# kamimrcht/ELECTOR

Measured on NVIDIA B200. Metric: triplets_per_sec, higher is better.
Workload: dtype s16x2 (packed halfword integer SIMD; int32 for scores beyond 16 bits)

## Files before the change

elector_b200/csrc/poa_dual.cuh:

```cuda
#pragma once
#include "poa_kernel.cuh"
#include "poa_packed.cuh"

namespace elector {

EL_HD uint32_t pk_select(uint32_t fresh, uint32_t old, uint32_t take) { return (fresh & take) | (old & ~take); }
EL_HD uint32_t pk_prmt(uint32_t a, uint32_t b, uint32_t sel) {
#ifdef __CUDA_ARCH__
  uint32_t r;
  asm("prmt.b32 %0, %1, %2, %3;" : "=r"(r) : "r"(a), "r"(b), "r"(sel));
  return r;
#else
  const uint64_t ab = ((uint64_t)b << 32) | a;
  uint32_t r = 0;
  for (int i = 0; i < 4; ++i) {
    const uint32_t n = (sel >> (4 * i)) & 0xfu;
    uint32_t byte = (uint32_t)(ab >> (8 * (n & 7u))) & 0xffu;
    if (n & 8u) byte = (byte & 0x80u) ? 0xffu : 0u;
    r |= byte << (8 * i);
  }
  return r;
#endif
}

enum : uint32_t { NM_REF = 1u << 7, NM_COR = 1u << 15, NM_MERGE = 1u << 23, NM_FINAL = 1u, NM_REFWINS = 2u };

struct Phase2D : Phase2<false> {
  static constexpr int kSetWords = 1;
  static EL_HD void put_row0(uint32_t *p, int bS, int bG) { p[R2_BS * 32] = pk2(kBiasP + bS, kBiasP + bG); }
  static EL_HD void put_shape(uint32_t *p, uint32_t ra) {
    p[R2_BG * 32] = ((ra & NF_REF) ? NM_REF : 0u) | ((ra & NF_COR) ? NM_COR : 0u) | ((ra & (NF_VIRT | NF_TWO)) ? NM_MERGE : 0u) |
                    ((ra & NF_FINAL) ? NM_FINAL : 0u) | (((ra & NF_VIRT) && !(ra & NF_PREDC)) ? NM_REFWINS : 0u) | ((ra & 0xffu) << 24);
  }
  EL_HDN int prepare(const uint16_t *nodes, int nx) const { return prepare_nodes(*this, nodes, nx); }

  template <int R, bool REF_SECOND>
  static EL_HD void merge(uint32_t (&Sr)[R], uint32_t (&Gr)[R], const uint32_t (&Sc)[R], const uint32_t (&Gc)[R], uint32_t &hr, uint32_t hc,
                          uint32_t take, uint32_t &oM, uint32_t &oX) {
    const uint32_t hm = REF_SECOND ? pk_maxs_flag(hc, hr, oM, 1u, 0u) : pk_maxs_flag(hr, hc, oM, 1u, 0u);
    if (take & 0xffffu) hr = hm;
#pragma unroll
    for (int k = 0; k < R; ++k) {
      const uint32_t bMl = 4u << (2 * k), bMh = R + k + 1 < kBand ? 4u << (2 * (R + k)) : 0u;
      const uint32_t bXl = 1u << (2 * k), bXh = 1u << (2 * (R + k));
      const uint32_t ms = REF_SECOND ? pk_maxs_flag(Sc[k], Sr[k], oM, bMl, bMh) : pk_maxs_flag(Sr[k], Sc[k], oM, bMl, bMh);
      const uint32_t mx = REF_SECOND ? pk_maxs_flag(Gc[k], Gr[k], oX, bXl, bXh) : pk_maxs_flag(Gr[k], Gc[k], oX, bXl, bXh);
      Sr[k] = pk_select(ms, Sr[k], take);
      Gr[k] = pk_select(mx, Gr[k], take);
    }
  }

  template <int R>
  EL_HDN void band(int nx, int ly, int b, bool last, int &best, int &best_j) const {
    constexpr uint32_t kLowMoves = ~0u << (32 - 2 * R);
    constexpr uint32_t kLowOrdM = (4u << (2 * R)) - 1u;
    constexpr uint32_t kLowOrdX = (1u << (2 * R)) - 1u;
    const int r0 = b * kBand;
    PackedConsts pc;
    pc.set(sc);
    uint32_t y2[R], Sr[R], Gr[R], Sc[R], Gc[R];
#pragma unroll
    for (int k = 0; k < R; ++k) {
      y2[k] = ((uint32_t)fs.code_at(Lp->f_unc, r0 + k) | ((uint32_t)fs.code_at(Lp->f_unc, r0 + R + k) << 16)) * 0x0101u;
      Sr[k] = Sc[k] = pk2(kBiasP + sc.virt_S(r0 + k), kBiasP + sc.virt_S(r0 + R + k));
      Gr[k] = Gc[k] = pk2(kBiasP + sc.virt_G(r0 + k), kBiasP + sc.virt_G(r0 + R + k));
    }
    uint32_t hr = (uint32_t)(kBiasP + sc.virt_S(r0 - 1)), hc = hr;
    const int rr = ly - 1 - r0;
    const bool lowrow = rr < R;
    uint32_t *p = rec(0);
    const int32_t step = (int32_t)(Lp->rec_words * 32);
    const int32_t o_bs = (int32_t)(R2_BS * 32) - step, o_mv = (int32_t)((R2_MOVES + (uint32_t)b) * 32) - step;
    uint32_t mr = 0, mc = 0, mg = 0, x2 = 0, nm_h = 0;
    uint32_t d7 = 0, g7 = 0, mlo = 0, ordM_lo = 0, ordX_lo = 0;
    uint32_t nm = p[R2_BG * 32], bsg = p[R2_BS * 32];
    uint32_t nm_n = p[step + R2_BG * 32], bsg_n = p[step + R2_BS * 32];
    for (int j = 0; j <= nx; ++j, p += step) {
      const uint32_t nm_n2 = p[2 * step + R2_BG * 32], bsg_n2 = p[2 * step + R2_BS * 32];
      if (j >= nx) nm = 0;
      mr = pk_prmt(mr, nm, 0x10ccu);
      mc = pk_prmt(mc, nm, 0x10ddu);
      mg = pk_prmt(mg, nm, 0x10eeu);
      x2 = pk_prmt(x2, nm, 0x1077u);
      if (mg) {
        const bool low = mg & 0xffffu;
        const uint32_t ram = low ? 0u : (p - step)[R2_NODE * 32];
        uint32_t oM = 0, oX = 0;
        if ((low ? nm : nm_h) & NM_REFWINS) merge<R, true>(Sr, Gr, Sc, Gc, hr, hc, mg, oM, oX);
        else merge<R, false>(Sr, Gr, Sc, Gc, hr, hc, mg, oM, oX);
        if (mg & 0xffffu) { ordM_lo = oM & kLowOrdM; ordX_lo = oX & kLowOrdX; }
        else {
          uint32_t *po = scr.at(Lp->o_ord + ((ram >> NF_SLOT_SHIFT) * Lp->ord_bands + (uint32_t)b) * 2);
          po[0] = ordM_lo | (oM & ~kLowOrdM);
          po[32] = ordX_lo | (oX & ~kLowOrdX);
        }
      }
      const uint32_t diag0 = pk_prmt(pk_select(hr, hc, mr), d7, 0x5410u);
      const uint32_t up0 = pk_prmt(bsg, g7, 0x5432u);
      d7 = pk_select(Sr[R - 1], Sc[R - 1], mr);
      uint32_t mv = 0, diag = diag0, up = up0, s = 0, g = 0;
#pragma unroll
      for (int k = 0; k < R; ++k) {
        const uint32_t pS = pk_select(Sr[k], Sc[k], mr), pG = pk_select(Gr[k], Gc[k], mr);
        const uint32_t t = pk_minu(x2 ^ y2[k], pc.mis2);
        const uint32_t M = diag - t;
        const uint32_t gap = pk_maxs_flag(up, pG, mv, 1u << (2 * (kBand - 1 - k)), 1u << (2 * (kBand - 1 - R - k)));
        s = pk_maxs_flag(gap, M, mv, 2u << (2 * (kBand - 1 - k)), 2u << (2 * (kBand - 1 - R - k)));
        g = pk_addmaxs(M, pc.nopen2, gap - pc.ext2);
        Sr[k] = pk_select(s, Sr[k], mr); Sc[k] = pk_select(s, Sc[k], mc);
        Gr[k] = pk_select(g, Gr[k], mr); Gc[k] = pk_select(g, Gc[k], mc);
        diag = pS; up = g;
      }
      g7 = g;
      hr = pk_select(bsg, hr, mr);
      hc = pk_select(bsg, hc, mc);
      if (j > 0) {
        if (!last) p[o_bs] = pk_prmt(s, g, 0x7632u);
        st_stream(p + o_mv, (mlo & kLowMoves) | (mv & ~kLowMoves));
      }
      mlo = mv;
      if (last && ((lowrow ? nm : nm_h) & NM_FINAL)) {
        const int kk = lowrow ? rr : rr - R;
        uint32_t v = pk_select(Sr[0], Sc[0], mr);
#pragma unroll
        for (int k = 1; k < R; ++k) if (kk == k) v = pk_select(Sr[k], Sc[k], mr);
        const int sf = (int)(lowrow ? v & 0xffffu : v >> 16) - kBiasP;
        if (sf > best) { best = sf; best_j = lowrow ? j : j - 1; }
      }
      nm_h = nm;
      nm = nm_n; bsg = bsg_n;
      nm_n = nm_n2; bsg_n = bsg_n2;
    }
  }

  mutable const uint16_t *p1n = nullptr;
  EL_HDN int fuse_emit(const AlignBits &al, int n1, int lu, const RowSink &out) const {
    const uint8_t *sym = sc.tab->sym;
    int col = 0, ix = 0, iy = 0;
    uint32_t w0 = 0, w1 = 0, w2 = 0;
    uint32_t ra0 = n1 > 0 ? p1n[0] : 0u, ra1 = n1 > 1 ? p1n[1] : 0u, ra2 = n1 > 2 ? p1n[2] : 0u, ra3 = n1 > 3 ? p1n[3] : 0u;
    while (ix < n1 || iy < lu) {
      const bool two = ix + 1 < n1 && (ra1 & NF_SAMERING);
      const bool xa = ix < n1 && (al.x_at(ix) || (two && al.x_at(ix + 1)));
      const bool ya = iy < lu && ((fs.w(al.oy + (uint32_t)(iy >> 5)) >> (iy & 31)) & 1u);
      const bool yonly = iy < lu && !ya && (ix >= n1 || xa);
      const bool takey = yonly || xa;
      const uint32_t rb = two ? (ra0 | ra1) : ra0;
      const uint32_t rl = (ra0 & NF_REF) ? ra0 : ra1, cl = (ra0 & NF_COR) ? ra0 : ra1;
      const uint32_t rc = (rb & NF_REF) ? (uint32_t)sym[rl & 31u] : (uint32_t)'.';
      const uint32_t cc = (rb & NF_COR) ? (uint32_t)sym[cl & 31u] : (uint32_t)'.';
      const uint32_t yc = sym[(fs.w(Lp->f_unc + (uint32_t)(iy >> 2)) >> ((iy & 3) * 8)) & 31u];
      const int sh = (col & 3) * 8;
      w0 |= (yonly ? (uint32_t)'.' : rc) << sh;
      w1 |= (yonly ? (uint32_t)'.' : cc) << sh;
      w2 |= (takey ? yc : (uint32_t)'.') << sh;
      if ((col & 3) == 3) { st_stream(out.r0 + (col >> 2), w0); st_stream(out.r1 + (col >> 2), w1); st_stream(out.r2 + (col >> 2), w2); w0 = w1 = w2 = 0; }
      ++col;
      iy += takey;
      if (!yonly) {
        const int adv = two ? 2 : 1;
        ix += adv;
        if (two) { ra0 = ra2; ra1 = ra3; ra2 = ix + 2 < n1 ? p1n[ix + 2] : 0u; ra3 = ix + 3 < n1 ? p1n[ix + 3] : 0u; }
        else { ra0 = ra1; ra1 = ra2; ra2 = ra3; ra3 = ix + 3 < n1 ? p1n[ix + 3] : 0u; }
      }
    }
    if (col & 3) { st_stream(out.r0 + (col >> 2), w0); st_stream(out.r1 + (col >> 2), w1); st_stream(out.r2 + (col >> 2), w2); }
    return col;
  }

  EL_HDN int dp(int nx, int ly, int &best_j) const {
    const int nb = (ly + kBand - 1) / kBand;
    int best = -999999;
    best_j = -1;
    for (int b = 0; b < nb - 1; ++b) band<8>(nx, ly, b, false, best, best_j);
    if (ly - (nb - 1) * kBand <= 8) band<4>(nx, ly, nb - 1, true, best, best_j);
    else band<8>(nx, ly, nb - 1, true, best, best_j);
    return best;
  }

  EL_HDN int align_window(const uint16_t *p1, int n1, const uint8_t *unc, int lu, int &s2, AlignBits &al) const {
    p1n = p1;
    for (int k = 0; k < n1; k += 64) prefetch_l1(p1 + k);
    fs.pack_codes(sc.tab, unc, lu, Lp->f_unc);
    EL_TICK(*this, 1);
    const int nrings = prepare(p1, n1);
    EL_TICK(*this, 2);
    int bj;
    s2 = dp(n1, lu, bj);
    EL_TICK(*this, 3);
    traceback(n1, lu, bj, al);
    EL_TICK(*this, 4);
    return columns_of(nrings, lu, al.nmatch);
  }
};

}
```

elector_b200/csrc/poa_kernel.cuh:

```cuda
#pragma once
#include <cuda_runtime.h>
#include <stddef.h>
#include <stdint.h>

namespace elector {

constexpr int kBand = 16;

#define EL_WARP_FULL 0xffffffffu
#define EL_HD __host__ __device__ __forceinline__
#define EL_HDN __host__ __device__

EL_HD uint32_t cdiv_u(uint32_t a, uint32_t b) { return (a + b - 1) / b; }
EL_HD uint32_t max_u(uint32_t a, uint32_t b) { return a > b ? a : b; }

enum : uint32_t { R1_BS = 0, R1_BG = 1, R1_MOVES = 2 };
enum : uint32_t { R2_NODE = 0, R2_BS = 1, R2_BG = 2, R2_PRED = 3, R2_MOVES = 4 };

struct Layout1 {
  uint32_t o_nodes;
  uint32_t rec_words;
  uint32_t o_fast;
  uint32_t f_ref, f_cor;
  uint32_t f_xb, f_yb;
// ... 29 lines not shown
}
EL_HD void make_layout2(Layout2 &L, int N1, int LU) {
  const uint32_t nb = cdiv_u(LU, kBand);
  uint32_t f = 0;
  L.f_unc = f; f += cdiv_u(LU, 4) + 4;
  L.f_xb = f; f += cdiv_u(N1, 32) + 1;
  L.f_yb = f; f += cdiv_u(LU, 32) + 1;
  L.f_nt = f; f += cdiv_u(N1, 32) + 1;
  L.f_total = f;
  uint32_t o = 0;
  L.rec_words = R2_MOVES + nb;
  L.o_nodes = o; o += ((uint32_t)N1 + 1) * L.rec_words;
  L.ord_bands = nb;
  L.o_ord = o; o += ((uint32_t)N1 / 2 + 2) * nb * 2;
  L.o_tmp = o; o += cdiv_u(N1, 4) + 1;
  L.o_fast = o; o += f;
  L.total = o;
}

struct PoaArgs {
  const uint8_t *ref, *cor, *unc;
  const int64_t *ref_off, *cor_off, *unc_off;
  const struct BinTable *tab;
  int32_t seg;
  const int32_t *items_base;
  uint32_t *scratch_base;
  int32_t *ctrl;
  const long long *rows_cap_dev;
  int32_t match, mismatch, open, ext;
  uint32_t mis2, nopen2, ext2;
  uint32_t arena_words;
  uint16_t *p1_nodes;
  int64_t ro0, co0;
  int32_t *n1;
  int32_t *key2;
  int32_t *hist2;
  int32_t *seg2_max;
  uint8_t *rows_out;
  unsigned long long *rows_cursor;
  int64_t rows_cap;
  int64_t *row_off;
  int32_t *row_stride, *nring, *score1, *score2;
  int64_t *cells;
  int32_t *error_flag;
  int32_t band_w;
  int32_t band_span;
};

struct SymbolTables {
  uint8_t code_lut[256];
  uint8_t sym[32];
  int16_t sub[32 * 32];
};

enum : uint32_t {
  NF_REF = 1u << 8,
  NF_COR = 1u << 9,
  NF_INITIAL = 1u << 10,
  NF_FINAL = 1u << 11,
  NF_SAMERING = 1u << 12,
  NF_KEEP = 0x1fffu,
  NF_VIRT = 1u << 13,
  NF_TWO = 1u << 14,
  NF_NOPRED = 1u << 15,
  NF_PREDC = 1u << 16,
  NF_SLOT_SHIFT = 17
};

constexpr int kBigTiers = 8;
constexpr int kSmallMax = 256;
constexpr int kNbMax = kSmallMax / 8;
constexpr int kN1q = 128;
constexpr int kSpCodes = 98;
constexpr int kSmallBins2 = kNbMax * kN1q * kSpCodes;
constexpr int kDcls = 4;
constexpr int kLinBins2 = kNbMax * kN1q * kDcls;
constexpr int kNumBins2 = kBigTiers + kSmallBins2 + kLinBins2;
constexpr int kNumSegs2 = kBigTiers + 8;
constexpr int kFirstLinSeg2 = kBigTiers + 4;

EL_HD int big_tier(int mx) {
  int t = 1;
  while ((kSmallMax << t) < mx && t < kBigTiers) ++t;
  return t;
}
EL_HD int seg2_of_nb(int nb8) { return kBigTiers + (nb8 > 16 ? 0 : nb8 > 8 ? 1 : nb8 > 4 ? 2 : 3); }
EL_HD void bin2_of(int n1, int lu, int spcode, bool linear, int &bin, int &seg) {
  if (lu > kSmallMax || n1 >= 4 * kN1q) {
    const int t = big_tier(n1 > lu ? n1 : lu);
    bin = seg = kBigTiers - t;
  } else {
    const int nb8 = (lu + 7) >> 3;
    if (linear) {
      int dc = (lu - n1 + 6) >> 2;
      dc = dc < 0 ? 0 : dc > kDcls - 1 ? kDcls - 1 : dc;
      const int lin = ((nb8 - 1) * kN1q + (n1 >> 2)) * kDcls + dc;
      bin = kBigTiers + kSmallBins2 + (kLinBins2 - 1 - lin);
      seg = seg2_of_nb(nb8) + 4;
    } else {
      const int small = ((nb8 - 1) * kN1q + (n1 >> 2)) * kSpCodes + spcode;
      bin = kBigTiers + (kSmallBins2 - 1 - small);
      seg = seg2_of_nb(nb8);
    }
  }
}

EL_HD int64_t p1_offset(int64_t ref_off, int64_t cor_off, int64_t w) { return (ref_off + cor_off + 8 * w) & ~(int64_t)3; }

EL_HD uint32_t shift_in_sign(uint32_t mv, int t) {
#ifdef __CUDA_ARCH__
  return __funnelshift_l((uint32_t)t, mv, 1);
#else
  return (mv << 1) | ((uint32_t)t >> 31);
#endif
}

#ifdef EL_DP_CLOCKS
__device__ unsigned long long g_dp_clk[2][8];
struct PhaseClock {
  mutable long long prev = 0;
  int kind = 0;
  __host__ __device__ void tick(int ph) const {
#ifdef __CUDA_ARCH__
    if ((threadIdx.x & 31) == 0) { const long long t = clock64(); atomicAdd(&g_dp_clk[kind][ph], (unsigned long long)(t - prev)); prev = t; }
#else
    (void)ph;
#endif
  }
};
#define EL_TICK(obj, ph) (obj).pclk.tick(ph)
#else
#define EL_TICK(obj, ph) ((void)0)
#endif

struct Scoring {
  const SymbolTables *tab;
  int match, mismatch, open, ext;
  uint32_t mis2, nopen2, ext2;
  EL_HD void set(int m, int mm, int o, int e) {
    match = m; mismatch = mm; open = o; ext = e;
    mis2 = ((uint32_t)(-mm) & 0xffffu) * 0x10001u; nopen2 = ((uint32_t)(-o) & 0xffffu) * 0x10001u; ext2 = ((uint32_t)e & 0xffffu) * 0x10001u;
  }
  EL_HD int virt_S(int row) const { return row < 0 ? 0 : -(open + ext * row); }
  EL_HD int virt_G(int row) const { return row < 0 ? -open : -(open + ext * row) - ext; }
};

constexpr int kBandMaxSpan = 500;
constexpr int kBandMaxScore = 7000;
EL_HD int band_span_limit(int maxabs) { const int s = kBandMaxScore / (maxabs > 0 ? maxabs : 1) - 4; return s < kBandMaxSpan ? s : kBandMaxSpan; }
struct BandW {
  int omin, omax;
  int w;
  bool on;
};
EL_HD int band_bound(const Scoring &sc, int w, int d) { return -(2 * sc.open + sc.ext * (2 * w + (d < 0 ? -d : d) - 2)); }



template <int R, bool GENERIC_SUB>
EL_HD uint32_t update_column(const Scoring &sc, int (&S)[R], int (&G)[R], const uint32_t (&yw)[R / 4], int xl, int diag, int up) {
  uint32_t mv = 0;
  const uint32_t x4 = (uint32_t)xl * 0x01010101u;
#pragma unroll
  for (int r = 0; r < R; ++r) {
    const int pS = S[r], pG = G[r];
    int sub;
    if (GENERIC_SUB) sub = (int)sc.tab->sub[xl * 32 + ((yw[r >> 2] >> ((r & 3) * 8)) & 31)];
    else sub = ((x4 ^ yw[r >> 2]) & (0xffu << ((r & 3) * 8))) ? sc.mismatch : sc.match;
    const int M = diag + sub;
    const int gap = pG > up ? pG : up;
    const bool isM = M > gap;
    const int s = isM ? M : gap;
    const int g = s - (isM ? sc.open : sc.ext);
    mv = shift_in_sign(mv, gap - M);
    mv = shift_in_sign(mv, up - pG);
    S[r] = s; G[r] = g;
    diag = pS; up = g;
  }
  if (R < kBand) mv <<= 2 * (kBand - R);
  return mv;
}

template <int R>
EL_HD int pick_row(const int (&S)[R], int k) {
  int s = S[0];
#pragma unroll
  for (int r = 1; r < R; ++r) if (k == r) s = S[r];
  return s;
}

struct LaneScratch {
  uint32_t *base;
  EL_HD uint32_t &w(uint32_t i) const { return base[(size_t)i * 32]; }
  EL_HD uint32_t *at(uint32_t i) const { return base + (size_t)i * 32; }
  EL_HD int code_at(uint32_t off, int i) const { return (w(off + (i >> 2)) >> ((i & 3) * 8)) & 0xff; }
  EL_HDN void pack_codes(const SymbolTables *tab, const uint8_t *src, int len, uint32_t off) const {
    const uintptr_t a = reinterpret_cast<uintptr_t>(src);
    const uint32_t *wp = reinterpret_cast<const uint32_t *>(a & ~(uintptr_t)3);
    const int mis = (int)(a & 3), sh = mis * 8;
    const int nin = (len + mis + 3) >> 2;
    const int nout = (len + 3) >> 2;
    const uint8_t *lut = tab->code_lut;
    uint32_t cur = wp[0];
#pragma unroll 1
    for (int k = 0; k < nout; k += 4) {
      uint32_t in[4];
#pragma unroll
      for (int i = 0; i < 4; ++i) in[i] = k + 1 + i < nin ? wp[k + 1 + i] : 0;
#pragma unroll
      for (int i = 0; i < 4; ++i) {
        const uint32_t nxt = in[i];
        if (k + i < nout) {
          const uint32_t v = sh ? (cur >> sh) | (nxt << (32 - sh)) : cur;
          uint32_t c = (uint32_t)lut[v & 0xff] | ((uint32_t)lut[(v >> 8) & 0xff] << 8) | ((uint32_t)lut[(v >> 16) & 0xff] << 16) |
                       ((uint32_t)lut[v >> 24] << 24);
          if (k + i == nout - 1 && (len & 3)) c &= 0xffffffffu >> (8 * (4 - (len & 3)));
          w(off + k + i) = c;
        }
        cur = nxt;
      }
    }
  }
};

EL_HD void prefetch_l1(const void *p) {
#ifdef __CUDA_ARCH__
  asm volatile("prefetch.global.L1 [%0];" ::"l"(p));
#else
  (void)p;
#endif
}
EL_HD void st_stream(uint32_t *p, uint32_t v) {
#ifdef __CUDA_ARCH__
  __stcs(p, v);
#else
  *p = v;
#endif
}

struct AlignBits {
  LaneScratch st;
  uint32_t ox, oy;
  int nmatch = 0;
  EL_HD void clear(int nx, int ny) const {
    for (uint32_t k = 0; k < cdiv_u((uint32_t)nx, 32); ++k) st.w(ox + k) = 0;
    for (uint32_t k = 0; k < cdiv_u((uint32_t)ny, 32); ++k) st.w(oy + k) = 0;
  }
  EL_HD void mark(int j, int r) {
    st.w(ox + (uint32_t)(j >> 5)) |= 1u << (j & 31);
    st.w(oy + (uint32_t)(r >> 5)) |= 1u << (r & 31);
    ++nmatch;
  }
  EL_HD bool x_at(int j) const { return (st.w(ox + (uint32_t)(j >> 5)) >> (j & 31)) & 1u; }
};
struct RowSink {
  uint32_t *r0, *r1, *r2;
};

EL_HDN inline int fuse1(const LaneScratch &cd, uint32_t o_ref, uint32_t o_cor, const AlignBits &al, int lr, int lc,
                      uint16_t *out, int &spcode) {
  int n = 0, ix = 0, iy = 0, sp = -1, sptype = 0;
  uint64_t *out4 = reinterpret_cast<uint64_t *>(out);
  uint64_t acc = 0;
  auto put = [&](uint32_t v) {
    acc |= (uint64_t)(v & 0xffffu) << (16 * (n & 3));
    if ((n & 3) == 3) { out4[n >> 2] = acc; acc = 0; }
    ++n;
  };
  while (ix < lr || iy < lc) {
    const bool xa = ix < lr && ((al.st.w(al.ox + (uint32_t)(ix >> 5)) >> (ix & 31)) & 1u);
    const bool ya = iy < lc && ((al.st.w(al.oy + (uint32_t)(iy >> 5)) >> (iy & 31)) & 1u);
    const bool yonly = iy < lc && !ya && (ix >= lr || xa);
    const uint32_t xl = (cd.w(o_ref + (uint32_t)(ix >> 2)) >> ((ix & 3) * 8)) & 0xffu;
    const uint32_t yl = (cd.w(o_cor + (uint32_t)(iy >> 2)) >> ((iy & 3) * 8)) & 0xffu;
    const uint32_t yf = NF_COR | (iy == 0 ? NF_INITIAL : 0u) | (iy == lc - 1 ? NF_FINAL : 0u);
    const bool diff = !yonly && xa && yl != xl;
    if (yonly || diff) {
      if (sp < 0) { sp = n; sptype = yonly ? 2 : 1; }
      put(yl | yf);
    }
    if (!yonly) {
      if (!xa && sp < 0) { sp = n; sptype = 0; }
      put(xl | NF_REF | (ix == 0 ? NF_INITIAL : 0u) | (ix == lr - 1 ? NF_FINAL : 0u) | (xa && !diff ? yf : 0u) | (diff ? NF_SAMERING : 0u));
    }
    ix += !yonly; iy += yonly || xa;
  }
  if (n & 3) out4[n >> 2] = acc;
  spcode = sp < 0 ? 0 : 1 + 3 * ((sp >> 1) < 31 ? (sp >> 1) : 31) + sptype;
  return n;
}

template <bool GENERIC_SUB>
struct Phase1 {
  typedef Layout1 Layout;
  static constexpr bool kGenericSub = GENERIC_SUB;
  static constexpr bool kBanded = false;
  static EL_HD void make_layout(Layout1 &L, int LR, int LC) { make_layout1(L, LR, LC); }
  LaneScratch scr;
  LaneScratch fs;
  Scoring sc;
  const Layout1 *Lp;

  template <int R>
  EL_HDN int band(int lr, int ly, int b, bool last) const {
    const int r0 = b * kBand;
    uint32_t yw[R / 4];
#pragma unroll
    for (int k = 0; k < R / 4; ++k) yw[k] = fs.w(Lp->f_cor + (r0 >> 2) + k);
// ... 230 lines not shown
template <bool GENERIC_SUB>
struct Phase2 {
  typedef Layout2 Layout;
  static constexpr bool kGenericSub = GENERIC_SUB;
  static constexpr bool kLinear = false;
  static constexpr bool kBanded = false;
  static constexpr int kSetWords = kSlotWords;
  static EL_HD void make_layout(Layout2 &L, int N1, int LU) { make_layout2(L, N1, LU); }
  LaneScratch scr;
  LaneScratch fs;
  uint32_t *bset;
  Scoring sc;
  const Layout2 *Lp;
#ifdef EL_DP_CLOCKS
  PhaseClock pclk;
#endif

  EL_HD uint32_t *rec(uint32_t j) const { return scr.at(Lp->o_nodes + j * Lp->rec_words); }

  static EL_HD void put_row0(uint32_t *p, int bS, int bG) { p[R2_BS * 32] = (uint32_t)bS; p[R2_BG * 32] = (uint32_t)bG; }
  static EL_HD void put_shape(uint32_t *, uint32_t) {}
  EL_HDN int prepare(const uint16_t *nodes, int nx) const { return prepare_nodes(*this, nodes, nx); }

  template <int R>
  EL_HDN void band(int nx, int ly, int b, bool last, int &best, int &best_j) const {
    const int r0 = b * kBand;
    uint32_t yw[R / 4];
#pragma unroll
    for (int k = 0; k < R / 4; ++k) yw[k] = fs.w(Lp->f_unc + (r0 >> 2) + k);
    int S[R], G[R], h = 0;
#pragma unroll
    for (int r = 0; r < R; ++r) S[r] = G[r] = 0;
    int kindA = 0, kindB = 0;
    int bsel = 0;
    uint32_t *p = rec(0);
    const uint32_t step = Lp->rec_words * 32;
    uint32_t ra = p[R2_NODE * 32];
    int upS = (int)p[R2_BS * 32], upG = (int)p[R2_BG * 32];
    for (int j = 0; j < nx; ++j, p += step) {
      const uint32_t *pn = j + 1 < nx ? p + step : p;
      const uint32_t ra_n = pn[R2_NODE * 32];
      const int upS_n = (int)pn[R2_BS * 32], upG_n = (int)pn[R2_BG * 32];

      const int m = (ra >> 8) & 3;
      if ((ra & (NF_TWO | NF_NOPRED | NF_VIRT | NF_PREDC)) || kindA != m) {
        uint32_t *sa = bset + (1 - bsel) * kSlotWords, *sb = bset + bsel * kSlotWords;
#pragma unroll
        for (int r = 0; r < R; ++r) { sa[r * 32] = (uint32_t)S[r]; sa[(R + r) * 32] = (uint32_t)G[r]; }
        sa[2 * R * 32] = (uint32_t)h;
        uint32_t *po = nullptr;
        if (ra & (NF_VIRT | NF_TWO)) po = scr.at(Lp->o_ord + ((ra >> NF_SLOT_SHIFT) * Lp->ord_bands + (uint32_t)b) * 2);
        const uint32_t st = arrange_sets(sa, sb, R, r0, ra, kindA, kindB, sc.open, sc.ext, po);
        kindA = st & 3; kindB = (st >> 2) & 3;
        if (st & 16u) { bsel = 1 - bsel; sa = sb; }
#pragma unroll
        for (int r = 0; r < R; ++r) { S[r] = (int)sa[r * 32]; G[r] = (int)sa[(R + r) * 32]; }
        h = (int)sa[2 * R * 32];
      }
      const uint32_t mv = update_column<R, GENERIC_SUB>(sc, S, G, yw, ra & 0xff, h, upG);
      h = upS;
      if (!last) { p[R2_BS * 32] = (uint32_t)S[R - 1]; p[R2_BG * 32] = (uint32_t)G[R - 1]; }
      p[(R2_MOVES + b) * 32] = mv;
      if (last && (ra & NF_FINAL)) {
        const int s = pick_row<R>(S, ly - 1 - r0);
        if (s > best) { best = s; best_j = j; }
      }
      ra = ra_n; upS = upS_n; upG = upG_n;
    }
  }

  EL_HDN int dp(int nx, int ly, int &best_j) const {
    const int nb = (ly + kBand - 1) / kBand;
    int best = -999999;
    best_j = -1;
    for (int b = 0; b < nb - 1; ++b) band<kBand>(nx, ly, b, false, best, best_j);
    if (ly - (nb - 1) * kBand <= 8) band<8>(nx, ly, nb - 1, true, best, best_j);
    else band<kBand>(nx, ly, nb - 1, true, best, best_j);
    return best;
  }

  EL_HDN void traceback(int nx, int ly, int best_j, AlignBits &al) const {
    const ptrdiff_t step = (ptrdiff_t)Lp->rec_words * 32;
    al.clear(nx, ly);
    int j = best_j, r = ly - 1, nmatch = 0;
    while (j >= 0 && r >= 0) {
      const int b = r >> 4;
      const uint32_t *p = rec((uint32_t)j);
      const uint32_t *pm = p + (R2_MOVES + b) * 32;
      const uint32_t w0 = *pm;
      if (j >= 6) prefetch_l1(pm - 6 * step);
      if (b > 0 && j >= 2) prefetch_l1(pm - 2 * step - 32);
      const uint32_t kind = (w0 >> (2 * (15 - (r & 15)))) & 3u;
      if (kind & 2u) {
        al.st.w(al.ox + (uint32_t)(j >> 5)) |= 1u << (j & 31);
        al.st.w(al.oy + (uint32_t)(r >> 5)) |= 1u << (r & 31);
        ++nmatch;
      }
      if (kind) {
        if ((fs.w(Lp->f_nt + (uint32_t)(j >> 5)) >> (j & 31)) & 1u) {
          const uint32_t ra = p[R2_NODE * 32];
          int ord = 0;
          if (ra & (NF_VIRT | NF_TWO)) {
            const uint32_t *po = scr.at(Lp->o_ord + ((ra >> NF_SLOT_SHIFT) * Lp->ord_bands + (uint32_t)b) * 2);
            ord = (int)((((kind & 2u) ? po[0] : po[32]) >> (2 * (r & 15))) & 3u);
          }
          const uint32_t pr = p[R2_PRED * 32];
          const int pA = (pr & 0xffffu) == 0xffffu ? -1 : (int)(pr & 0xffffu), pB = (pr >> 16) == 0xffffu ? -1 : (int)(pr >> 16);
          if (ra & NF_VIRT) j = (ord == 0) ? -1 : (ord == 1 ? pA : pB);
          else j = (ord == 0) ? pA : pB;
        } else --j;
      }
      if (kind != 1u) --r;
    }
    al.nmatch = nmatch;
  }

  static constexpr uint32_t kRecNode = R2_NODE, kRecPred = R2_PRED;
  EL_HD uint32_t *node_rec(int j) const { return rec((uint32_t)j); }
  EL_HD uint32_t node_flags(const uint32_t *rec_j, int) const { return rec_j[R2_NODE * 32]; }
  EL_HDN int fuse_emit(const AlignBits &al, int n1, int lu, const RowSink &out) const { return fuse_emit_rows(*this, al, n1, lu, out); }
  EL_HD AlignBits bits() const { return AlignBits{fs, Lp->f_xb, Lp->f_yb}; }

  EL_HDN int align_window(const uint16_t *p1, int n1, const uint8_t *unc, int lu, int &s2, AlignBits &al) const {
    fs.pack_codes(sc.tab, unc, lu, Lp->f_unc);
    EL_TICK(*this, 1);
    const int nrings = prepare(p1, n1);
    EL_TICK(*this, 2);
    int bj;
    s2 = dp(n1, lu, bj);
    EL_TICK(*this, 3);
    traceback(n1, lu, bj, al);
    EL_TICK(*this, 4);
    return columns_of(nrings, lu, al.nmatch);
  }
};

#ifndef EL_MIN_WARPS_PH1
#define EL_MIN_WARPS_PH1 28
#endif
#ifndef EL_MIN_WARPS_PH2
#define EL_MIN_WARPS_PH2 20
#endif

template <bool GENERIC_SUB>
__device__ __forceinline__ const SymbolTables *stage_tables(uint32_t *smem, const SymbolTables *g_tab) {
  constexpr int kTabWords = (GENERIC_SUB ? sizeof(SymbolTables) : offsetof(SymbolTables, sub)) / 4;
  const uint32_t *s = reinterpret_cast<const uint32_t *>(g_tab);
  for (int i = threadIdx.x; i < kTabWords; i += 32) smem[i] = s[i];
  __syncwarp();
  return reinterpret_cast<const SymbolTables *>(smem);
}

#ifdef __CUDACC__
__device__ __forceinline__ void group_band(BandW &bw, bool on, int w, bool active, int d) {
  const int lo = active ? (d < 0 ? d : 0) : 0, hi = active ? (d > 0 ? d : 0) : 0;
  bw.omin = __reduce_min_sync(EL_WARP_FULL, lo) - w;
  bw.omax = __reduce_max_sync(EL_WARP_FULL, hi) + w;
  bw.w = w;
  bw.on = on;
}
__device__ __forceinline__ bool queue_retries(int32_t *queue, int &nretry, bool failed, int w) {
  const unsigned fm = __ballot_sync(EL_WARP_FULL, failed);
  if (fm == 0) return false;
  const int lane = threadIdx.x & 31;
  if (failed) queue[nretry + __popc(fm & ((1u << lane) - 1u))] = w;
  nretry += __popc(fm);
  __syncwarp();
  if (nretry < 32) return false;
  nretry -= 32;
  return true;
}

__device__ __forceinline__ void warp_hist_add(int32_t *hist, int bin) {
  const unsigned peers = __match_any_sync(__activemask(), bin);
  if ((int)(threadIdx.x & 31) == __ffs(peers) - 1) atomicAdd(&hist[bin], __popc(peers));
}

__device__ __forceinline__ void phase1_epilogue(const PoaArgs &a, bool active, int w, int n1, int s1, int spcode, int lr, int lc) {
  (void)lr; (void)lc;
  if (active) {
    const int lu = (int)(a.unc_off[w + 1] - a.unc_off[w]);
    int bin, seg;
    bin2_of(n1, lu, spcode, false, bin, seg);
    a.n1[w] = n1;
    a.key2[w] = bin;
    if (a.score1) a.score1[w] = s1;
    warp_hist_add(a.hist2, bin);
    if (n1 > a.seg2_max[seg * 4]) atomicMax(&a.seg2_max[seg * 4], n1);
    if (lu > a.seg2_max[seg * 4 + 1]) atomicMax(&a.seg2_max[seg * 4 + 1], lu);
  }
}
#endif

struct SegRun {
  const int32_t *items;
  int32_t n_items;
  uint32_t warp_words;
  uint32_t *scratch;
  int32_t *work_counter;
  long long rows_cap;
};
__device__ __forceinline__ bool seg_setup(const PoaArgs &a, SegRun &run);

extern __shared__ uint32_t s_arena[];
template <class L>
__device__ __forceinline__ uint32_t *fast_base(const PoaArgs &a, const L &layout, uint32_t *lane_scratch, int lane) {
  return layout.f_total <= a.arena_words ? s_arena + lane : lane_scratch + (size_t)layout.o_fast * 32;
}

template <class PH, int MIN_WARPS>
__global__ void __launch_bounds__(32, MIN_WARPS) poa_dp1_kernel(PoaArgs a, const SymbolTables *g_tab) {
  constexpr bool GENERIC_SUB = PH::kGenericSub;
  __shared__ uint32_t s_tab[(GENERIC_SUB ? sizeof(SymbolTables) : offsetof(SymbolTables, sub)) / 4];
  __shared__ typename PH::Layout s_layout;
  const int lane = threadIdx.x;
  __shared__ SegRun s_run;
  if (!seg_setup(a, s_run)) return;
  PH c;
  c.scr.base = s_run.scratch + (size_t)blockIdx.x * s_run.warp_words * 32 + lane;
  c.sc.tab = stage_tables<GENERIC_SUB>(s_tab, g_tab);
  c.sc.match = a.match; c.sc.mismatch = a.mismatch; c.sc.open = a.open; c.sc.ext = a.ext;
  c.sc.mis2 = a.mis2; c.sc.nopen2 = a.nopen2; c.sc.ext2 = a.ext2;
  c.Lp = &s_layout;
  __shared__ int32_t s_retry[64];
  int nretry = 0;
  auto process = [&](int w, bool active, bool banded) -> bool {
    int lr = 0, lc = 0;
    int64_t ro = 0, co = 0;
    if (active) {
      ro = a.ref_off[w]; co = a.cor_off[w];
      lr = (int)(a.ref_off[w + 1] - ro); lc = (int)(a.cor_off[w + 1] - co);
    }
    {
      const int mr = __reduce_max_sync(EL_WARP_FULL, lr), mc = __reduce_max_sync(EL_WARP_FULL, lc);
      __syncwarp();
      if (lane == 0) PH::make_layout(s_layout, mr, mc);
      __syncwarp();
      if constexpr (PH::kBanded) group_band(c.bw, banded && mr + mc <= a.band_span, a.band_w + (mc >> 4), active, lc - lr);
    }
    if (s_layout.total > s_run.warp_words) { if (lane == 0) atomicExch(a.error_flag, 2); return false; }
    c.fs.base = fast_base(a, s_layout, c.scr.base, lane);
    int s1 = 0, spcode = 0, n1 = 0;
    bool exact = true;
    if (active) n1 = c.run_window(a.ref + ro, lr, a.cor + co, lc, a.p1_nodes + p1_offset(ro - a.ro0, co - a.co0, w), s1, spcode, exact);
    phase1_epilogue(a, active && exact, w, n1, s1, spcode, lr, lc);
    __syncwarp();
    return active && !exact;
  };
  for (;;) {
    int base = 0;
    if (lane == 0) base = atomicAdd(s_run.work_counter, 32);
    base = __shfl_sync(EL_WARP_FULL, base, 0);
    if (base >= s_run.n_items) break;
    const bool active = base + lane < s_run.n_items;
    const int w = active ? s_run.items[base + lane] : -1;
    const bool failed = process(w, active, a.band_w > 0);
    if constexpr (PH::kBanded) {
      if (queue_retries(s_retry, nretry, failed, w)) { const int w2 = s_retry[nretry + lane]; __syncwarp(); process(w2, true, false); }
    }
  }
  if constexpr (PH::kBanded) {
    if (nretry > 0) { const bool act = lane < nretry; const int w2 = act ? s_retry[lane] : -1; __syncwarp(); process(w2, act, false); }
  }
}

#ifdef __CUDACC__
__device__ __forceinline__ bool alloc_window_rows(const PoaArgs &a, long long rows_cap, bool active, int w, int nring, RowSink &out) {
  const int lane = threadIdx.x;
  const int stride = active ? (nring + 3) & ~3 : 0;
  const int bytes = 3 * stride;
  int incl = bytes;
  for (int d = 1; d < 32; d <<= 1) {
    const int t = __shfl_up_sync(EL_WARP_FULL, incl, d);
    if (lane >= d) incl += t;
  }
  const int total = __shfl_sync(EL_WARP_FULL, incl, 31);
  unsigned long long wbase = 0;
  if (lane == 0 && total) wbase = atomicAdd(a.rows_cursor, (unsigned long long)total);
  wbase = __shfl_sync(EL_WARP_FULL, wbase, 0);
  if (!active) return false;
  const int64_t off = (int64_t)wbase + incl - bytes;
  a.row_off[w] = off;
  a.row_stride[w] = stride;
  if (off + bytes > rows_cap) { atomicExch(a.error_flag, 1); return false; }
  out.r0 = reinterpret_cast<uint32_t *>(a.rows_out + off);
  out.r1 = out.r0 + (stride >> 2);
  out.r2 = out.r1 + (stride >> 2);
  return true;
}

#endif
template <class PH, int MIN_WARPS>
__global__ void __launch_bounds__(32, MIN_WARPS) poa_dp2_kernel(PoaArgs a, const SymbolTables *g_tab) {
  constexpr bool GENERIC_SUB = PH::kGenericSub;
  __shared__ uint32_t s_tab[(GENERIC_SUB ? sizeof(SymbolTables) : offsetof(SymbolTables, sub)) / 4];
  __shared__ typename PH::Layout s_layout;
  __shared__ uint32_t s_bset[2 * PH::kSetWords];
  const int lane = threadIdx.x;
  __shared__ SegRun s_run;
  if (!seg_setup(a, s_run)) return;
  PH c;
  c.scr.base = s_run.scratch + (size_t)blockIdx.x * s_run.warp_words * 32 + lane;
  c.bset = s_bset + lane;
  c.sc.tab = stage_tables<GENERIC_SUB>(s_tab, g_tab);
  c.sc.match = a.match; c.sc.mismatch = a.mismatch; c.sc.open = a.open; c.sc.ext = a.ext;
  c.sc.mis2 = a.mis2; c.sc.nopen2 = a.nopen2; c.sc.ext2 = a.ext2;
  c.Lp = &s_layout;
  __shared__ int32_t s_retry[64];
  int nretry = 0;
  auto process = [&](int w, bool active, bool banded) -> bool {
    int nring = 0, n1 = 0, lu = 0;
    int64_t ro = 0, co = 0, uo = 0;
    if (active) {
      ro = a.ref_off[w]; co = a.cor_off[w]; uo = a.unc_off[w];
      lu = (int)(a.unc_off[w + 1] - uo);
      n1 = a.n1[w];
    }
    {
      const int mn = __reduce_max_sync(EL_WARP_FULL, n1), mu = __reduce_max_sync(EL_WARP_FULL, lu);
      __syncwarp();
      if (lane == 0) PH::make_layout(s_layout, mn, mu);
      __syncwarp();
      if constexpr (PH::kBanded) group_band(c.bw, banded && mn + mu <= a.band_span, a.band_w + (mu >> 3), active, lu - n1);
    }
    if (s_layout.total > s_run.warp_words) { if (lane == 0) atomicExch(a.error_flag, 2); return false; }
    c.fs.base = fast_base(a, s_layout, c.scr.base, lane);
    bool exact = true;
    AlignBits al = c.bits();
    EL_TICK(c, 0);
    if (active) {
      int s2;
      if constexpr (PH::kLinear) nring = c.align_linear(a.ref + ro, n1, a.unc + uo, lu, s2, exact, al);
      else nring = c.align_window(a.p1_nodes + p1_offset(ro - a.ro0, co - a.co0, w), n1, a.unc + uo, lu, s2, al);
      if (exact) {
        a.nring[w] = nring;
        if (a.score2) a.score2[w] = s2;
        if (a.cells) {
          const int64_t lr = a.ref_off[w + 1] - ro, lc = a.cor_off[w + 1] - co;
          a.cells[w] = lr * lc + (int64_t)n1 * lu;
        }
      } else nring = 0;
    }
    __syncwarp();
    RowSink out;
    if (alloc_window_rows(a, s_run.rows_cap, active && exact, w, nring, out)) c.fuse_emit(al, n1, lu, out);
    __syncwarp();
    EL_TICK(c, 5);
    return active && !exact;
  };
#ifdef EL_DP_CLOCKS
  c.pclk.kind = PH::kLinear ? 0 : 1;
  c.pclk.prev = clock64();
#endif
  for (;;) {
    int base = 0;
    if (lane == 0) base = atomicAdd(s_run.work_counter, 32);
    base = __shfl_sync(EL_WARP_FULL, base, 0);
    if (base >= s_run.n_items) break;
    const bool active = base + lane < s_run.n_items;
    const int w = active ? s_run.items[base + lane] : -1;
    const bool failed = process(w, active, a.band_w > 0);
    if constexpr (PH::kBanded) {
      if (queue_retries(s_retry, nretry, failed, w)) { const int w2 = s_retry[nretry + lane]; __syncwarp(); process(w2, true, false); }
    }
  }
  if constexpr (PH::kBanded) {
    if (nretry > 0) { const bool act = lane < nretry; const int w2 = act ? s_retry[lane] : -1; __syncwarp(); process(w2, act, false); }
  }
}

}
```

elector_b200/csrc/poa_packed.cuh:

```cuda
#pragma once
#include "poa_kernel.cuh"

namespace elector {

constexpr int kBiasP = 16384;
constexpr int kNegP = kBiasP - 8000;
constexpr int kPackedSpan = 16000;

EL_HD int packed_rows(int ly) {
  const int nb = (ly + 15) >> 4;
  const int need = (ly + 2 * nb - 1) / (2 * nb);
  return need <= 6 ? 6 : need <= 7 ? 7 : 8;
}

EL_HD uint32_t pk_minu(uint32_t a, uint32_t b) {
#ifdef __CUDA_ARCH__
  return __vminu2(a, b);
#else
  const uint32_t al = a & 0xffffu, bl = b & 0xffffu, ah = a >> 16, bh = b >> 16;
  return (al < bl ? al : bl) | ((ah < bh ? ah : bh) << 16);
#endif
}
EL_HD uint32_t pk_maxs_flag(uint32_t a, uint32_t b, uint32_t &mv, uint32_t bit_lo, uint32_t bit_hi) {
#ifdef __CUDA_ARCH__
  uint32_t val;
  asm("{.reg .pred pu, pv;\n\t"
      ".reg .s16 rs0, rs1, rs2, rs3;\n\t"
      "max.s16x2 %0, %2, %3;\n\t"
      "mov.b32 {rs0, rs1}, %0;\n\t"
      "mov.b32 {rs2, rs3}, %2;\n\t"
      "setp.eq.s16 pv, rs0, rs2;\n\t"
      "setp.eq.s16 pu, rs1, rs3;\n\t"
      "@!pv or.b32 %1, %1, %4;\n\t"
      "@!pu or.b32 %1, %1, %5;}\n\t"
      : "=&r"(val), "+r"(mv) : "r"(a), "r"(b), "r"(bit_lo), "r"(bit_hi));
  return val;
#else
  const int16_t al = (int16_t)(a & 0xffffu), bl = (int16_t)(b & 0xffffu), ah = (int16_t)(a >> 16), bh = (int16_t)(b >> 16);
  if (bl > al) mv |= bit_lo;
  if (bh > ah) mv |= bit_hi;
  return (uint32_t)(uint16_t)(al >= bl ? al : bl) | ((uint32_t)(uint16_t)(ah >= bh ? ah : bh) << 16);
#endif
}
EL_HD uint32_t pk_addmaxs(uint32_t a, uint32_t b, uint32_t c) {
#ifdef __CUDA_ARCH__
  return __viaddmax_s16x2(a, b, c);
#else
  const int16_t sl = (int16_t)((a + b) & 0xffffu), sh = (int16_t)(((a >> 16) + (b >> 16)) & 0xffffu);
  const int16_t cl = (int16_t)(c & 0xffffu), ch = (int16_t)(c >> 16);
  return (uint32_t)(uint16_t)(sl > cl ? sl : cl) | ((uint32_t)(uint16_t)(sh > ch ? sh : ch) << 16);
#endif
}
EL_HD uint32_t pk2(int lo, int hi) { return ((uint32_t)lo & 0xffffu) | ((uint32_t)hi << 16); }
EL_HD uint32_t pk_lo_hi(uint32_t lo_src, uint32_t hi_src) {
  return (lo_src & 0xffffu) | (hi_src & 0xffff0000u);
}

struct PackedConsts {
  uint32_t mis2, nopen2, ext2;
  EL_HD void set(const Scoring &sc) {
    mis2 = sc.mis2; nopen2 = sc.nopen2; ext2 = sc.ext2;
  }
};

template <int R>
EL_HD uint32_t update_packed(const PackedConsts &pc, uint32_t (&S)[R], uint32_t (&G)[R], const uint32_t (&y2)[R], uint32_t x2,
                             uint32_t diag, uint32_t up) {
  uint32_t mv = 0;
#pragma unroll
  for (int k = 0; k < R; ++k) {
    const uint32_t pS = S[k], pG = G[k];
    const uint32_t t = pk_minu(x2 ^ y2[k], pc.mis2);
    const uint32_t M = diag - t;
    const uint32_t gap = pk_maxs_flag(up, pG, mv, 1u << (2 * k), 1u << (16 + 2 * k));
    const uint32_t s = pk_maxs_flag(gap, M, mv, 2u << (2 * k), 2u << (16 + 2 * k));
    const uint32_t g = pk_addmaxs(M, pc.nopen2, gap - pc.ext2);
    S[k] = s; G[k] = g;
    diag = pS; up = g;
  }
  return mv;
}

template <int R>
EL_HD int pick_half(const uint32_t (&S)[R], int k, bool hi) {
  uint32_t s = S[0];
#pragma unroll
  for (int r = 1; r < R; ++r) if (k == r) s = S[r];
  return (int)(hi ? s >> 16 : s & 0xffffu) - kBiasP;
}

enum : uint32_t { P1_BSG = 0, P1_MOVES = 1 };

struct Layout1P {
  uint32_t o_nodes, rec_words, R;
  uint32_t o_fast, f_ref, f_cor, f_xb, f_yb, f_total;
  uint32_t total;
};
EL_HD void make_layout1p(Layout1P &L, int LR, int LC) {
  uint32_t f = 0;
  L.f_ref = f; f += cdiv_u(LR, 4) + 3;
  L.f_cor = f; f += cdiv_u(LC, 4) + 5;
  L.f_xb = f; f += cdiv_u(LR, 32) + 1;
  L.f_yb = f; f += cdiv_u(LC, 32) + 1;
  L.f_total = f;
  uint32_t o = 0;
  L.R = (uint32_t)packed_rows(LC);
  L.rec_words = P1_MOVES + cdiv_u(LC, 16);
  L.o_nodes = o; o += ((uint32_t)LR + 4) * L.rec_words;
  L.o_fast = o; o += f;
  L.total = o;
}

struct Phase1P {
  typedef Layout1P Layout;
  static constexpr bool kGenericSub = false;
  static constexpr bool kBanded = true;
  LaneScratch scr;
  LaneScratch fs;
  Scoring sc;
  const Layout1P *Lp;
  BandW bw = {0, 0, 0, false};
  static EL_HD void make_layout(Layout1P &L, int LR, int LC) { make_layout1p(L, LR, LC); }

  EL_HD uint32_t *rec(int j) const { return scr.at(Lp->o_nodes + (uint32_t)(j + 1) * Lp->rec_words); }
  EL_HD bool band_exact(int score, int lx, int ly) const {
    if (!bw.on) return true;
    const int bound = band_bound(sc, bw.w, ly - lx);
    return score > bound && bound > kNegP - kBiasP;
  }

  template <int R>
  EL_HDN int band(int lr, int ly, int b, bool last, const BandW &bw) const {
    const int r0 = b * 2 * R;
    PackedConsts pc;
    pc.set(sc);
    int jlo = 0, jend = lr;
    if (bw.on) {
      jlo = r0 - bw.omax > 0 ? r0 - bw.omax : 0;
      const int jhi = r0 + 2 * R - 1 - bw.omin;
      jend = jhi + 1 < lr ? jhi + 1 : lr;
      if (jlo > jend) jlo = jend;
    }
    uint32_t y2[R], S[R], G[R];
#pragma unroll
    for (int k = 0; k < R; ++k) {
      y2[k] = ((uint32_t)fs.code_at(Lp->f_cor, r0 + k) | ((uint32_t)fs.code_at(Lp->f_cor, r0 + R + k) << 16)) << 4;
      const int v = kBiasP + sc.virt_S(r0 + k);
      S[k] = (uint32_t)v;
      G[k] = (uint32_t)(v - sc.ext);
      if (jlo > 0) S[k] = G[k] = pk2(kNegP, kNegP);
    }
    const int rr = ly - 1 - r0;
    uint32_t *p = rec(jlo - 1);
    const uint32_t step = Lp->rec_words * 32;
    uint32_t bsg, bsg_n, bsg_n2 = 0;
    if (b == 0) {
      bsg = pk2(kBiasP, kBiasP - sc.open);
      bsg_n = pk2(kBiasP - sc.open, kBiasP - sc.open - sc.ext);
    } else {
      bsg = p[P1_BSG * 32];
      bsg_n = p[step + P1_BSG * 32];
      bsg_n2 = p[2 * step + P1_BSG * 32];
    }
    uint32_t xw = 0, xw_next = fs.w(Lp->f_ref + (jlo >> 2)), x2 = 0, d7 = 0, mlo = 0;
    if (jlo > 0) { x2 = (uint32_t)fs.code_at(Lp->f_ref, jlo - 1) << 4; d7 = (uint32_t)kNegP; }
    int best = 0;
    for (int j = jlo; j <= jend; ++j, p += step) {
      if ((j & 3) == 0 || j == jlo) { xw = xw_next >> (8 * (j & 3)); xw_next = fs.w(Lp->f_ref + (j >> 2) + 1); }
      x2 = (x2 << 16) | ((xw & 0xffu) << 4);
      xw >>= 8;
      const uint32_t bsg_p = bsg;
      bsg = bsg_n;
      if (b == 0) bsg_n = bsg - pc.ext2;
      else { bsg_n = bsg_n2; bsg_n2 = p[3 * step + P1_BSG * 32]; }
      const uint32_t diag0 = pk_lo_hi(bsg_p, d7 << 16);
      const uint32_t up0 = (bsg >> 16) | (G[R - 1] << 16);
      d7 = S[R - 1];
      const uint32_t mv = update_packed<R>(pc, S, G, y2, x2, diag0, up0);
      if (!last) p[P1_BSG * 32] = (S[R - 1] >> 16) | (G[R - 1] & 0xffff0000u);
      st_stream(p + (P1_MOVES + b) * 32, pk_lo_hi(mlo, mv));
      mlo = mv;
      if (last && j == lr - 1 && rr < R) best = pick_half<R>(S, rr, false);
    }
    if (last && rr >= R) best = pick_half<R>(S, rr - R, true);
    if (bw.on && !last) {
      const int stop = jend + 2 * R + 3 < lr + 2 ? jend + 2 * R + 3 : lr + 2;
      for (int j = jend; j <= stop; ++j, p += step) p[P1_BSG * 32] = pk2(kNegP, kNegP);
    }
    return best;
  }

  template <int R>
  EL_HDN int dp(int lr, int ly, const BandW &bw) const {
    const int nb = (ly + 2 * R - 1) / (2 * R);
    for (int b = 0; b < nb - 1; ++b) band<R>(lr, ly, b, false, bw);
    return band<R>(lr, ly, nb - 1, true, bw);
  }

  template <int R>
  EL_HDN void traceback(int lr, int ly, AlignBits &al) const {
    al.clear(lr, ly);
    const uint32_t *base = rec(0) + P1_MOVES * 32;
    const int rw = (int)Lp->rec_words;
    int j = lr - 1, r = ly - 1;
    int b = r / (2 * R), rr = r - b * 2 * R;
    int nmatch = 0;
    while (j >= 0 && r >= 0) {
      const uint32_t *pm = base + (ptrdiff_t)(j * rw + b) * 32;
      const uint32_t w = *pm;
      if (j >= 6) prefetch_l1(pm - (ptrdiff_t)6 * rw * 32);
      if (b > 0 && j >= 2) prefetch_l1(pm - (ptrdiff_t)2 * rw * 32 - 32);
      const uint32_t kind = (w >> (rr < R ? 2 * rr : 16 + 2 * (rr - R))) & 3u;
      if (kind & 2u) {
        al.st.w(al.ox + (uint32_t)(j >> 5)) |= 1u << (j & 31);
        al.st.w(al.oy + (uint32_t)(r >> 5)) |= 1u << (r & 31);
        ++nmatch;
      }
      const int dr = kind != 1u, dj = kind != 0u;
      j -= dj; r -= dr; rr -= dr;
      if (rr < 0) { rr += 2 * R; --b; }
    }
    al.nmatch = nmatch;
  }

  template <int R>
  EL_HDN int run_r(int lr, int lc, uint16_t *p1_out, int &s1, int &spcode, bool &exact) const {
    s1 = dp<R>(lr, lc, bw);
    exact = band_exact(s1, lr, lc);
    if (!exact) return 0;
    AlignBits al{fs, Lp->f_xb, Lp->f_yb};
    traceback<R>(lr, lc, al);
    return fuse1(fs, Lp->f_ref, Lp->f_cor, al, lr, lc, p1_out, spcode);
  }

  EL_HDN void pack(const uint8_t *x, int lx, const uint8_t *y, int ly) const {
    fs.pack_codes(sc.tab, x, lx, Lp->f_ref);
    fs.pack_codes(sc.tab, y, ly, Lp->f_cor);
    for (uint32_t k = 0; k < 5; ++k) fs.w(Lp->f_cor + cdiv_u((uint32_t)ly, 4) + k) = 0;
    fs.w(Lp->f_ref + cdiv_u((uint32_t)lx, 4)) = 0;
    fs.w(Lp->f_ref + cdiv_u((uint32_t)lx, 4) + 1) = 0;
  }

  EL_HDN int run_window(const uint8_t *ref, int lr, const uint8_t *cor, int lc, uint16_t *p1_out, int &s1, int &spcode, bool &exact) const {
    pack(ref, lr, cor, lc);
    if (Lp->R == 6) return run_r<6>(lr, lc, p1_out, s1, spcode, exact);
    if (Lp->R == 7) return run_r<7>(lr, lc, p1_out, s1, spcode, exact);
    return run_r<8>(lr, lc, p1_out, s1, spcode, exact);
  }
};

struct Layout2L : Layout1P {};
EL_HD void make_layout2l(Layout2L &L, int N1, int LU) { make_layout1p(L, N1, LU); }

struct Phase2L {
  typedef Layout2L Layout;
  static constexpr bool kGenericSub = false;
  static constexpr bool kLinear = true;
  static constexpr bool kBanded = true;
  static constexpr int kSetWords = 1;
  static EL_HD void make_layout(Layout2L &L, int N1, int LU) { make_layout2l(L, N1, LU); }
  LaneScratch scr, fs;
  uint32_t *bset;
  Scoring sc;
  const Layout2L *Lp;
  BandW bw = {0, 0, 0, false};
#ifdef EL_DP_CLOCKS
  PhaseClock pclk;
#endif

  EL_HD AlignBits bits() const { return AlignBits{fs, Lp->f_xb, Lp->f_yb}; }
  EL_HD Phase1P core() const {
    Phase1P d;
    d.scr = scr; d.fs = fs; d.sc = sc; d.Lp = Lp; d.bw = bw;
    return d;
  }

  EL_HDN int fuse_emit(const AlignBits &al, int n1, int lu, const RowSink &out) const {
    const uint8_t *sym = sc.tab->sym;
    int col = 0, ix = 0, iy = 0;
    uint32_t w0 = 0, w2 = 0;
    while (ix < n1 || iy < lu) {
      const bool xa = ix < n1 && ((fs.w(al.ox + (uint32_t)(ix >> 5)) >> (ix & 31)) & 1u);
      const bool ya = iy < lu && ((fs.w(al.oy + (uint32_t)(iy >> 5)) >> (iy & 31)) & 1u);
      const bool yonly = iy < lu && !ya && (ix >= n1 || xa);
      const bool takey = yonly || xa;
      const uint32_t xc = sym[(fs.w(Lp->f_ref + (uint32_t)(ix >> 2)) >> ((ix & 3) * 8)) & 31u];
      const uint32_t yc = sym[(fs.w(Lp->f_cor + (uint32_t)(iy >> 2)) >> ((iy & 3) * 8)) & 31u];
      const int sh = (col & 3) * 8;
      w0 |= (yonly ? (uint32_t)'.' : xc) << sh;
      w2 |= (takey ? yc : (uint32_t)'.') << sh;
      if ((col & 3) == 3) { st_stream(out.r0 + (col >> 2), w0); st_stream(out.r1 + (col >> 2), w0); st_stream(out.r2 + (col >> 2), w2); w0 = w2 = 0; }
      ++col;
      ix += !yonly; iy += takey;
    }
    if (col & 3) { st_stream(out.r0 + (col >> 2), w0); st_stream(out.r1 + (col >> 2), w0); st_stream(out.r2 + (col >> 2), w2); }
// ... 26 lines not shown
```

Before: 1.656 million.

## Add diagonal banding with exactness check and retry to dual-graph POA phase

Extends banded DP to the Phase2D (dual ref/cor graph) aligner. Each row band now iterates only over a diagonal window of columns, with a skip allowance derived from merged-node counts. A bound check marks results as inexact and queues them for a full unbanded retry. The work loop is restructured so retries and leftovers go through one process call site, and a shared band_iters helper is factored out. The cost is the retry path and band-edge sentinel writes, and correctness depends on the band bound being sound.

After: 1.699 million (median of 6 runs). 1.03x the previous value.

```diff
diff --git a/elector_b200/csrc/poa_dual.cuh b/elector_b200/csrc/poa_dual.cuh
--- a/elector_b200/csrc/poa_dual.cuh
+++ b/elector_b200/csrc/poa_dual.cuh
@@ -27,6 +27,8 @@
 
 struct Phase2D : Phase2<false> {
   static constexpr int kSetWords = 1;
+  static constexpr bool kBanded = true;
+  BandW bw = {0, 0, 0, false};
   static EL_HD void put_row0(uint32_t *p, int bS, int bG) { p[R2_BS * 32] = pk2(kBiasP + bS, kBiasP + bG); }
   static EL_HD void put_shape(uint32_t *p, uint32_t ra) {
     p[R2_BG * 32] = ((ra & NF_REF) ? NM_REF : 0u) | ((ra & NF_COR) ? NM_COR : 0u) | ((ra & (NF_VIRT | NF_TWO)) ? NM_MERGE : 0u) |
@@ -50,12 +52,21 @@
     }
   }
 
+  EL_HD bool band_exact(int score, int nx, int ly) const {
+    if (!bw.on) return true;
+    const int d = ly - nx, dmin = d >= 0 ? d : d + bw.s >= 0 ? 0 : -(d + bw.s);
+    const int bound = band_bound(sc, bw.w, dmin);
+    return score > bound && bound > kNegP - kBiasP;
+  }
+
   template <int R>
   EL_HDN void band(int nx, int ly, int b, bool last, int &best, int &best_j) const {
     constexpr uint32_t kLowMoves = ~0u << (32 - 2 * R);
     constexpr uint32_t kLowOrdM = (4u << (2 * R)) - 1u;
     constexpr uint32_t kLowOrdX = (1u << (2 * R)) - 1u;
     const int r0 = b * kBand;
+    int jlo, jend;
+    band_iters(bw, r0, 2 * R, nx, jlo, jend);
     PackedConsts pc;
     pc.set(sc);
     uint32_t y2[R], Sr[R], Gr[R], Sc[R], Gc[R];
@@ -64,18 +75,24 @@
       y2[k] = ((uint32_t)fs.code_at(Lp->f_unc, r0 + k) | ((uint32_t)fs.code_at(Lp->f_unc, r0 + R + k) << 16)) * 0x0101u;
       Sr[k] = Sc[k] = pk2(kBiasP + sc.virt_S(r0 + k), kBiasP + sc.virt_S(r0 + R + k));
       Gr[k] = Gc[k] = pk2(kBiasP + sc.virt_G(r0 + k), kBiasP + sc.virt_G(r0 + R + k));
+      if (jlo > 0) Sr[k] = Sc[k] = Gr[k] = Gc[k] = pk2(kNegP, kNegP);
     }
     uint32_t hr = (uint32_t)(kBiasP + sc.virt_S(r0 - 1)), hc = hr;
     const int rr = ly - 1 - r0;
     const bool lowrow = rr < R;
-    uint32_t *p = rec(0);
+    uint32_t *p = rec((uint32_t)jlo);
     const int32_t step = (int32_t)(Lp->rec_words * 32);
+    if (jlo > 0) {
+      const uint32_t nm_p = (p - step)[R2_BG * 32], s_p = (p - step)[R2_BS * 32] & 0xffffu;
+      hr = (nm_p & NM_REF) ? s_p : (uint32_t)kNegP;
+      hc = (nm_p & NM_COR) ? s_p : (uint32_t)kNegP;
+    }
     const int32_t o_bs = (int32_t)(R2_BS * 32) - step, o_mv = (int32_t)((R2_MOVES + (uint32_t)b) * 32) - step;
     uint32_t mr = 0, mc = 0, mg = 0, x2 = 0, nm_h = 0;
     uint32_t d7 = 0, g7 = 0, mlo = 0, ordM_lo = 0, ordX_lo = 0;
     uint32_t nm = p[R2_BG * 32], bsg = p[R2_BS * 32];
     uint32_t nm_n = p[step + R2_BG * 32], bsg_n = p[step + R2_BS * 32];
-    for (int j = 0; j <= nx; ++j, p += step) {
+    for (int j = jlo; j <= jend; ++j, p += step) {
       const uint32_t nm_n2 = p[2 * step + R2_BG * 32], bsg_n2 = p[2 * step + R2_BS * 32];
       if (j >= nx) nm = 0;
       mr = pk_prmt(mr, nm, 0x10ccu);
@@ -131,6 +148,8 @@
       nm = nm_n; bsg = bsg_n;
       nm_n = nm_n2; bsg_n = bsg_n2;
     }
+    if (bw.on && !last)
+      for (int j = jend; j <= jend + kBand && j < nx; ++j) (p + (j - jend - 1) * step)[R2_BS * 32] = pk2(kNegP, kNegP);
   }
 
   mutable const uint16_t *p1n = nullptr;
@@ -178,7 +197,7 @@
     return best;
   }
 
-  EL_HDN int align_window(const uint16_t *p1, int n1, const uint8_t *unc, int lu, int &s2, AlignBits &al) const {
+  EL_HDN int align_window(const uint16_t *p1, int n1, const uint8_t *unc, int lu, int &s2, bool &exact, AlignBits &al) const {
     p1n = p1;
     for (int k = 0; k < n1; k += 64) prefetch_l1(p1 + k);
     fs.pack_codes(sc.tab, unc, lu, Lp->f_unc);
@@ -188,10 +207,16 @@
     int bj;
     s2 = dp(n1, lu, bj);
     EL_TICK(*this, 3);
+    exact = band_exact(s2, n1, lu);
+    if (!exact) return 0;
     traceback(n1, lu, bj, al);
     EL_TICK(*this, 4);
     return columns_of(nrings, lu, al.nmatch);
   }
+  EL_HDN int align_window(const uint16_t *p1, int n1, const uint8_t *unc, int lu, int &s2, AlignBits &al) const {
+    bool exact;
+    return align_window(p1, n1, unc, lu, s2, exact, al);
+  }
 };
 
 }
diff --git a/elector_b200/csrc/poa_kernel.cuh b/elector_b200/csrc/poa_kernel.cuh
--- a/elector_b200/csrc/poa_kernel.cuh
+++ b/elector_b200/csrc/poa_kernel.cuh
@@ -205,8 +205,18 @@
   int omin, omax;
   int w;
   bool on;
+  int s = 0;
 };
 EL_HD int band_bound(const Scoring &sc, int w, int d) { return -(2 * sc.open + sc.ext * (2 * w + (d < 0 ? -d : d) - 2)); }
+EL_HD void band_iters(const BandW &bw, int r0, int rows, int nx, int &jlo, int &jend) {
+  jlo = 0; jend = nx;
+  if (bw.on) {
+    jlo = r0 - bw.omax > 0 ? r0 - bw.omax : 0;
+    const int jhi = r0 + rows - 1 - bw.omin;
+    jend = jhi + 1 < nx ? jhi + 1 : nx;
+    if (jlo > jend) jlo = jend;
+  }
+}
 
 
 
@@ -743,12 +753,13 @@
 }
 
 #ifdef __CUDACC__
-__device__ __forceinline__ void group_band(BandW &bw, bool on, int w, bool active, int d) {
-  const int lo = active ? (d < 0 ? d : 0) : 0, hi = active ? (d > 0 ? d : 0) : 0;
+__device__ __forceinline__ void group_band(BandW &bw, bool on, int w, bool active, int d, int s = 0) {
+  const int lo = active ? (d < 0 ? d : 0) - s : 0, hi = active ? (d + s > 0 ? d + s : 0) : 0;
   bw.omin = __reduce_min_sync(EL_WARP_FULL, lo) - w;
   bw.omax = __reduce_max_sync(EL_WARP_FULL, hi) + w;
   bw.w = w;
   bw.on = on;
+  bw.s = s;
 }
 __device__ __forceinline__ bool queue_retries(int32_t *queue, int &nretry, bool failed, int w) {
   const unsigned fm = __ballot_sync(EL_WARP_FULL, failed);
@@ -912,7 +923,11 @@
       __syncwarp();
       if (lane == 0) PH::make_layout(s_layout, mn, mu);
       __syncwarp();
-      if constexpr (PH::kBanded) group_band(c.bw, banded && mn + mu <= a.band_span, a.band_w + (mu >> 3), active, lu - n1);
+      if constexpr (PH::kBanded) {
+        int skip = 0;
+        if (!PH::kLinear && active) skip = 2 * n1 - (int)(a.ref_off[w + 1] - ro) - (int)(a.cor_off[w + 1] - co);
+        group_band(c.bw, banded && mn + mu <= a.band_span, a.band_w + (mu >> 3), active, lu - n1, skip);
+      }
     }
     if (s_layout.total > s_run.warp_words) { if (lane == 0) atomicExch(a.error_flag, 2); return false; }
     c.fs.base = fast_base(a, s_layout, c.scr.base, lane);
@@ -922,6 +937,7 @@
     if (active) {
       int s2;
       if constexpr (PH::kLinear) nring = c.align_linear(a.ref + ro, n1, a.unc + uo, lu, s2, exact, al);
+      else if constexpr (PH::kBanded) nring = c.align_window(a.p1_nodes + p1_offset(ro - a.ro0, co - a.co0, w), n1, a.unc + uo, lu, s2, exact, al);
       else nring = c.align_window(a.p1_nodes + p1_offset(ro - a.ro0, co - a.co0, w), n1, a.unc + uo, lu, s2, al);
       if (exact) {
         a.nring[w] = nring;
@@ -943,21 +959,30 @@
   c.pclk.kind = PH::kLinear ? 0 : 1;
   c.pclk.prev = clock64();
 #endif
+  bool retry = false, rest = false;
   for (;;) {
-    int base = 0;
-    if (lane == 0) base = atomicAdd(s_run.work_counter, 32);
-    base = __shfl_sync(EL_WARP_FULL, base, 0);
-    if (base >= s_run.n_items) break;
-    const bool active = base + lane < s_run.n_items;
-    const int w = active ? s_run.items[base + lane] : -1;
-    const bool failed = process(w, active, a.band_w > 0);
-    if constexpr (PH::kBanded) {
-      if (queue_retries(s_retry, nretry, failed, w)) { const int w2 = s_retry[nretry + lane]; __syncwarp(); process(w2, true, false); }
-    }
-  }
-  if constexpr (PH::kBanded) {
-    if (nretry > 0) { const bool act = lane < nretry; const int w2 = act ? s_retry[lane] : -1; __syncwarp(); process(w2, act, false); }
-  }
-}
-
-}
+    int w = -1;
+    bool active = true;
+    if (retry) w = s_retry[nretry + lane];
+    else {
+      int base = 0;
+      if (lane == 0) base = atomicAdd(s_run.work_counter, 32);
+      base = __shfl_sync(EL_WARP_FULL, base, 0);
+      if (base < s_run.n_items) {
+        active = base + lane < s_run.n_items;
+        if (active) w = s_run.items[base + lane];
+      } else {
+        if (!PH::kBanded || nretry == 0) break;
+        rest = true;
+        active = lane < nretry;
+        if (active) w = s_retry[lane];
+      }
+    }
+    __syncwarp();
+    const bool failed = process(w, active, a.band_w > 0 && !retry && !rest);
+    if (rest) break;
+    retry = PH::kBanded && queue_retries(s_retry, nretry, failed, w);
+  }
+}
+
+}
diff --git a/elector_b200/csrc/poa_packed.cuh b/elector_b200/csrc/poa_packed.cuh
--- a/elector_b200/csrc/poa_packed.cuh
+++ b/elector_b200/csrc/poa_packed.cuh
@@ -134,13 +134,8 @@
     const int r0 = b * 2 * R;
     PackedConsts pc;
     pc.set(sc);
-    int jlo = 0, jend = lr;
-    if (bw.on) {
-      jlo = r0 - bw.omax > 0 ? r0 - bw.omax : 0;
-      const int jhi = r0 + 2 * R - 1 - bw.omin;
-      jend = jhi + 1 < lr ? jhi + 1 : lr;
-      if (jlo > jend) jlo = jend;
-    }
+    int jlo, jend;
+    band_iters(bw, r0, 2 * R, lr, jlo, jend);
     uint32_t y2[R], S[R], G[R];
 #pragma unroll
     for (int k = 0; k < R; ++k) {
```
